# lxjeffffff/PagedAttention-Based-Transformer-Decoder-Inference-Framework

Measured on AMD Instinct MI355X. Metric: decode tokens/sec at batch=64 seq_len=8192; % HBM-roofline (1/2/4/8 GPU), higher is better.
Workload: dtype int8 GEMM (i32 acc) + fp16 KV attention (fp32 acc); 1 GPU; C3: INT8 decoder (MFMA i8 matmuls + fp16 paged attention), 24-layer/16-head/d=128, batch 64, KV context 8192, page 16; strong scaling: 64 rows over 1 GPU(s); global_batch=64, batch_per_gpu=64, seq_len=8192, page_size=16, parallelism=single GPU (no collective)

## Files before the change

pagedattention-based-transformer-decoder-inference-framework_amd/csrc/decoder.cpp:

```cpp
#include <algorithm>
#include <cmath>
#include <memory>
#include <mutex>
#include <random>
#include <string>
#include <vector>

#include "decoder_impl.hpp"

static int check_cfg(const llm_decoder_config& c) {
  LLM_REQUIRE(c.num_layers > 0 && c.num_heads > 0 && c.head_dim > 0 && c.vocab_size > 0 &&
                  c.max_seq_len > 0,
              "decoder: num_layers/num_heads/head_dim/vocab_size/max_seq_len must be positive");
  LLM_REQUIRE(c.hidden_dim == c.num_heads * c.head_dim,
              "decoder: hidden_dim must equal num_heads * head_dim");
  LLM_REQUIRE(c.weight_dtype == LLM_I8 || c.weight_dtype == LLM_F16, "decoder: weight_dtype");
  return LLM_OK;
}

static int create_decoder(const llm_decoder_config* cfg_in, int kv_dtype, llm_decoder** out) {
  LLM_REQUIRE(cfg_in && out, "llm_decoder_create: NULL");
  LLM_REQUIRE(kv_elem_size(kv_dtype) > 0, "llm_decoder_create_kv: unknown kv_dtype");
  if (kv_dtype != LLM_F16 && kv_dtype != LLM_FP8)
    return fail(LLM_ERR_UNSUPPORTED, "llm_decoder_create_kv: the decoder's KV pools are LLM_F16 "
// ... 33 lines not shown
  RET_IF(d->lm_pi.alloc((size_t)B * d->lm_nwg));
  RET_IF(d->sa.alloc((size_t)B));
  const size_t B16 = ((size_t)B + 15) / 16 * 16;
  RET_IF(d->qa.alloc(B16 * std::max(hid, inter)));
  if (d->wdtype == LLM_F16) {
    RET_IF(d->a16.alloc(2 * B16 * std::max(hid, inter)));
    RET_IF(d->oacc.alloc((size_t)B * hid));
    LLM_HIP_RET(hipMemset(d->oacc.p, 0, sizeof(long long) * B * hid));
    RET_IF(d->oflag.alloc(2));
    LLM_HIP_RET(hipMemset(d->oflag.p, 0, 2 * sizeof(int)));
    LLM_HIP_RET(hipHostMalloc(reinterpret_cast<void**>(&d->h_oflag), sizeof(int)));
    *d->h_oflag = 0;
  }
  RET_IF(d->beam_ctr.alloc(2 * (((size_t)B + 3) / 4) * d->H));
  LLM_HIP_RET(hipMemset(d->beam_ctr.p, 0, sizeof(unsigned) * d->beam_ctr.n));
  d->b16 = B16;
  RET_IF(d->tokens.alloc((size_t)B));
  RET_IF(d->beam_score.alloc((size_t)B));
  RET_IF(d->beam_ws.alloc(beam_select_ws_floats(B, 4)));
  RET_IF(d->cand_score.alloc((size_t)2 * B));
  RET_IF(d->cand_parent.alloc((size_t)2 * B));
  RET_IF(d->cand_token.alloc((size_t)2 * B));
  RET_IF(d->pos.alloc((size_t)B));
  RET_IF(d->ctx.alloc((size_t)B));
  d->pps = 0;
  d->attn_ws_bytes = 16;
  for (int b = 1; b <= B; ++b)
    d->attn_ws_bytes = std::max(d->attn_ws_bytes,
                                pa_decode_workspace_bytes(b, d->H, d->D, d->max_tiles, 0));
  RET_IF(d->attn_ws.alloc(std::max<size_t>(d->attn_ws_bytes, 16)));
// ... 84 lines not shown
  delete d;
}

extern "C" kv_cache* llm_decoder_kv(llm_decoder* d) { return d ? d->kv : nullptr; }

int llm::reset_rows(llm_decoder* d, int batch, int start_pos) {
  LLM_REQUIRE(batch > 0 && batch <= d->maxB, "decoder: batch must be in [1, max_batch]");
  RET_IF(kv_cache_clear(d->kv));
  d->batch = batch;
  if (d->row_group != 1) d->drop_step_graph();
  d->row_group = 1;
  d->h_pos.assign(d->maxB, 0);
  for (int b = 0; b < batch; ++b) d->h_pos[b] = start_pos;
  if (d->oacc.p) LLM_HIP_RET(hipMemset(d->oacc.p, 0, sizeof(long long) * d->oacc.n));
  if (d->oflag.p) LLM_HIP_RET(hipMemset(d->oflag.p, 0, sizeof(int)));
  d->range_clamped = 0;
  std::vector<int32_t> pos(batch, start_pos), ctx(batch, start_pos + 1), tok(batch, 0);
  LLM_HIP_RET(hipMemcpy(d->pos.p, pos.data(), sizeof(int32_t) * batch, hipMemcpyHostToDevice));
  LLM_HIP_RET(hipMemcpy(d->ctx.p, ctx.data(), sizeof(int32_t) * batch, hipMemcpyHostToDevice));
  LLM_HIP_RET(hipMemcpy(d->tokens.p, tok.data(), sizeof(int32_t) * batch, hipMemcpyHostToDevice));
  LLM_HIP_RET(hipDeviceSynchronize());
  return LLM_OK;
}

static void shuffle_free_pages(KvCache* k, uint64_t seed) {
  std::lock_guard<std::mutex> gk(k->mu);
  std::mt19937_64 rng(seed ^ 7);
  for (auto& f : k->free_lists) std::shuffle(f.begin(), f.end(), rng);
}

// ... 223 lines not shown
```

pagedattention-based-transformer-decoder-inference-framework_amd/csrc/decoder_impl.hpp:

```cpp
#pragma once

#include <mutex>
#include <string>
#include <unordered_map>
#include <vector>

#include "common.hpp"
#include "gemm.hpp"
#include "kv_cache_impl.hpp"
#include "pa_decode.hpp"
#include "row_ops.hpp"
#include "serve_plan.hpp"

using namespace llm;

namespace llm {

template <typename T>
struct __attribute__((visibility("hidden"))) DevBuf {
  T* p = nullptr;
  size_t n = 0;
  ~DevBuf() { if (p) (void)hipFree(p); }
  int alloc(size_t count) {
    if (p) { (void)hipFree(p); p = nullptr; }
// ... 14 lines not shown

struct Rows {
  int n = 0;
  float* x = nullptr;
  float* q = nullptr;
  float* o = nullptr;
  float* h1 = nullptr;
  void* act = nullptr;
  void* act2 = nullptr;
  float* sa = nullptr;
  const int32_t* pos = nullptr;
  const int32_t* ctx = nullptr;
  const int32_t* beam_rows = nullptr;
  int row_group = 1;
  bool wgm_quant = false;
  int prefill_row = -1;
  int prefill_p0 = 0;
  const int32_t* prefill_tiles = nullptr;
  int prefill_ntile = 0;
  int prefill_maxend = 0;
  bool is_prefill() const { return prefill_row >= 0 || prefill_ntile > 0; }
  uint8_t* attn_ws = nullptr;
  size_t attn_ws_bytes = 0;
  long long* oacc = nullptr;
  float* oproj_out = nullptr;
  int* oflag = nullptr;
};

struct llm_decoder {
  llm_decoder_config cfg{};
// ... 18 lines not shown
  DevBuf<float> rope;
  bool rope_on = false;
  int window = 0;

  DevBuf<float> x, qkv, o, h1, logits, sa;
  DevBuf<float> lm_pv;
  DevBuf<int32_t> lm_pi;
  int lm_nwg = 0;
  DevBuf<int8_t> qa;
  DevBuf<uint16_t> a16;
  DevBuf<long long> oacc, oacc_run;
  DevBuf<int> oflag, oflag_run;
  int* h_oflag = nullptr;
  int range_clamped = 0;
  DevBuf<unsigned> beam_ctr;
  int oproj_range_status();
  int report_range(int flag);
  DevBuf<int32_t> tokens, pos, ctx;
  DevBuf<uint8_t> attn_ws;
  size_t attn_ws_bytes = 0;

  int batch = 0;
  std::vector<int> h_pos;

  hipGraphExec_t graph = nullptr;
  int graph_batch{-1};
  void drop_step_graph() { graph_batch = -1; }

  int8_t* tap_q = nullptr;
  float* tap_s = nullptr;
// ... 15 lines not shown
  uint64_t sample_seed = 0;
  bool use_graph = true;
  bool beam_mode = false;
  DevBuf<float> beam_score, beam_ws, cand_score;
  DevBuf<int32_t> cand_parent, cand_token;
  std::vector<int32_t> h_cand;
  int qa_ld = 0;
  size_t b16 = 0;

  int layer_pre(int l, hipStream_t st, const Rows& R, const LnSource* emb = nullptr);
  int layer_attn(int l, hipStream_t st, const Rows& R);
  int attn_request(const Rows& R, pa_kv_view* view, PaRequest* rq, int l = 0);
  bool quant_prologue(const Rows& R) const;
  bool oproj_fusable(const Rows& R);
  bool wgm_quant_ok(const Rows& R);
  bool fc2_split(const Rows& R) const;
  int layer_post(int l, hipStream_t st, const Rows& R);
  int decode_rows(Rows* R, bool scratch_oproj = false);
  int next_tokens(const float* xr, int n, int r0, const int32_t* ctr, hipStream_t st,
                  int32_t* adv_pos = nullptr, int32_t* adv_ctx = nullptr);
  int enqueue_step(hipStream_t st);
  int run_step(const int32_t* tokens_host, float* logits_dev, int32_t* next_host, hipStream_t st);

  static constexpr int kPrefillChunk = 512;
  DevBuf<float> px, pq, po, ph1, psa;
  DevBuf<uint8_t> pact, pws;
  DevBuf<int32_t> pmeta;
  size_t pws_bytes = 0;
  int pf_cap = 0;
  int prefill_reserve(int C);
// ... 45 lines not shown
```

pagedattention-based-transformer-decoder-inference-framework_amd/csrc/decoder_serve.cpp:

```cpp
#include <cmath>
#include <mutex>
#include <string>
#include <vector>

#include "decoder_impl.hpp"

int llm_decoder::serve_upload() {
  const int n = plan.live();
  for (int r = 0; r < n; ++r) {
    const llm_request_options& o = requests.at(plan.row(r).id).opt;
    hs_temp[r] = o.temperature;
    hs_topk[r] = o.top_k;
    hs_topp[r] = o.top_p;
    hs_seed[r] = o.seed;
    hs_pos[r] = h_pos[r];
    hs_ctx[r] = h_pos[r] + 1;
  }
  auto up = [&](void* dst, const void* src, size_t bytes) {
    return hipMemcpyAsync(dst, src, bytes * n, hipMemcpyHostToDevice, stream);
  };
  LLM_HIP_RET(up(sv_temp.p, hs_temp.data(), sizeof(float)));
  LLM_HIP_RET(up(sv_topk.p, hs_topk.data(), sizeof(int32_t)));
  LLM_HIP_RET(up(sv_topp.p, hs_topp.data(), sizeof(float)));
  LLM_HIP_RET(up(sv_seed.p, hs_seed.data(), sizeof(uint64_t)));
// ... 70 lines not shown
  std::lock_guard<std::mutex> g(d->mu);
  LLM_REQUIRE(!d->serving, "llm_decoder_serve_begin: already serving");
  LLM_REQUIRE(d->weights_ready, "llm_decoder_serve_begin: weights not loaded");
  if (d->beam_mode)
    return fail(LLM_ERR_UNSUPPORTED, "llm_decoder_serve_begin: the decoder is in beam mode");
  if (d->V > 65536)
    return fail(LLM_ERR_UNSUPPORTED, "llm_decoder_serve_begin: vocab_size > 65536 (the rows' "
                                     "tokens are chosen by sample_rows_each)");
  LLM_HIP_RET(hipStreamSynchronize(d->stream));
  RET_IF(kv_cache_clear(d->kv));
  d->batch = 0;
  d->row_group = 1;
  d->h_pos.assign(d->maxB, 0);
  if (d->oacc.p) LLM_HIP_RET(hipMemset(d->oacc.p, 0, sizeof(long long) * d->oacc.n));
  if (d->oflag.p) LLM_HIP_RET(hipMemset(d->oflag.p, 0, sizeof(int)));
  LLM_HIP_RET(hipDeviceSynchronize());
  d->range_clamped = 0;
  const size_t B = (size_t)d->maxB;
  if (!d->sv_temp.p) {
    RET_IF(d->sv_temp.alloc(B));
    RET_IF(d->sv_topk.alloc(B));
    RET_IF(d->sv_topp.alloc(B));
    RET_IF(d->sv_seed.alloc(B));
  }
  d->hs_temp.assign(B, 0.f); d->hs_topp.assign(B, 1.f); d->hs_topk.assign(B, 0);
  d->hs_seed.assign(B, 0); d->hs_pos.assign(B, 0); d->hs_ctx.assign(B, 1);
  d->hs_tok.assign(B, 0); d->hs_next.assign(B, 0);
  ServeGeom geom;
  geom.max_rows = d->maxB;
  geom.num_pages = kv_cache_num_pages(d->kv);
// ... 92 lines not shown
```

pagedattention-based-transformer-decoder-inference-framework_amd/csrc/decoder_step.cpp:

```cpp
#include <mutex>
#include <string>

#include "decoder_impl.hpp"

__global__ void take_flag_kernel(int* f) { f[1] = atomicExch(f, 0); }

int llm_decoder::layer_pre(int l, hipStream_t st, const Rows& R, const LnSource* emb) {
  const size_t lh = (size_t)l * hid;
  pa_kv_view view;
  RET_IF(kv_cache_view(kv, l, &view));
  KvAppendView app;
  app.pos = R.pos;
  app.page_table = view.page_table;
  app.rows = R.beam_rows;
  app.k_pool = kv_cache_k_pool(kv);
  app.v_pool = kv_cache_v_pool(kv);
  app.num_beams = view.num_beams;
  app.max_tiles = view.max_tiles;
  app.page_size = TS;
  app.num_pages = view.num_pages;
  app.H = H;
  app.D = D;
  app.page_stride = (size_t)view.page_stride / kv_elem_size(kvt);
  app.kv_dtype = kvt;
// ... 56 lines not shown
  return attn_request(r, &view, &rq) == LLM_OK && pa_plan_device(rq, &p) == LLM_OK && p.oproj;
}

bool llm_decoder::wgm_quant_ok(const Rows& R) {
  if (wdtype != LLM_I8 || R.is_prefill() || R.row_group != 1 || R.beam_rows ||
      quant_prologue(R))
    return false;
  Rows r = R;
  r.wgm_quant = true;
  pa_kv_view view;
  PaRequest rq;
  PaLaunch p;
  return attn_request(r, &view, &rq) == LLM_OK && pa_plan_device(rq, &p) == LLM_OK && p.wgm;
}

bool llm_decoder::fc2_split(const Rows& R) const {
  return wdtype == LLM_I8 && !R.is_prefill() &&
         (R.n <= 16 || (R.n > 32 && R.n <= 64 && inter >= 16384)) &&
         !ln_fusable(wdtype, R.n, hid) && inter / 64 >= 16;
}

int llm_decoder::attn_request(const Rows& R, pa_kv_view* view, PaRequest* rq, int l) {
  RET_IF(kv_cache_view(kv, l, view));
  const PaOut out = quant_prologue(R) || R.wgm_quant ? PaOut::F32_ROWS
                    : wdtype == LLM_I8               ? PaOut::ROW_Q
                    : R.oacc                         ? PaOut::OPROJ
                                                     : PaOut::ROW_F16;
  *rq = pa_request(view, R.n, H, D, cfg.max_seq_len, pps, R.row_group, out);
  rq->rows16 = out == PaOut::OPROJ && tap_q;
  rq->steal_ctr = R.row_group >= 4 && beam_steal_on();
  rq->window = window;
  return LLM_OK;
}

int llm_decoder::layer_attn(int l, hipStream_t st, const Rows& R) {
  pa_kv_view view;
  PaRequest rq;
  RET_IF(attn_request(R, &view, &rq, l));
  PaRowOutputs ro;
  ro.pack = 1;
  ro.keep_out = 0;
  if (rq.out == PaOut::ROW_Q) {
    ro.q = static_cast<int8_t*>(R.act);
    ro.inv_scale = R.sa;
  } else if (rq.out == PaOut::OPROJ) {
    ro.o_acc = R.oacc;
    ro.o_x = R.oproj_out;
    ro.wo_heads = wo_heads.p + (size_t)l * hid * hid;
    ro.o_n = hid;
    ro.o_flag = R.oflag;
    ro.out16 = rq.rows16 ? R.act : nullptr;
  } else if (rq.out == PaOut::ROW_F16) {
    ro.out16 = R.act;
  }
  if (rq.steal_ctr) ro.beam_ctr = beam_ctr.p;
  ro.out_scale = v_scale[l];
  const float sm = kvt == LLM_FP8 ? cfg.attn_scale * k_scale[l] : cfg.attn_scale;
  if (R.is_prefill() && pa_prefill_supported(&view)) {
    if (R.prefill_ntile > 0)
// ... 9 lines not shown
    LLM_HIP_RET(launch_quantize_rows(R.o, R.n, hid, static_cast<int8_t*>(R.act), R.sa, st, 1));
  return LLM_OK;
}

int llm_decoder::layer_post(int l, hipStream_t st, const Rows& R) {
  const size_t lh = (size_t)l * hid;
  const bool i8 = wdtype == LLM_I8;
  WeightGemm g;
  g.dtype = wdtype;
  g.a_packed = 1;
  g.w_keep = w_keep;
  g.A = R.act;
  g.M = R.n;
  g.W_packed = wo.p + sz_o * l; g.N = hid; g.K = hid; g.C = R.x;
  if (i8) { g.sa = R.sa; g.sw = sw_o.p + lh; }
  const bool qpro = quant_prologue(R);
  if (qpro) {
    g.ln_x = R.o;
    g.ln_quant_only = 1;
    if (tap_q) { g.act_out = R.act; g.sa_out = R.sa; }
  }
  if (!R.oacc) RET_IF(weight_gemm(g, st));
  g.ln_x = nullptr; g.ln_quant_only = 0; g.act_out = nullptr; g.sa_out = nullptr;
  RET_IF(tap(l, 1, R, hid, st));
  const bool split_fc2 = fc2_split(R);
  RET_IF(layer_norm_into(g, R, ln2_g.p + lh, ln2_b.p + lh, st, split_fc2 ? R.x : nullptr));
  g.W_packed = w1.p + sz_1 * l; g.N = inter; g.K = hid;
  g.bias = b1.p + (size_t)l * inter; g.act = LLM_ACT_RELU;
  if (i8) {
    g.C = R.h1;
    g.sw = sw1.p + (size_t)l * inter;
// ... 27 lines not shown
  R.ctx = ctx.p;
  R.row_group = row_group;
  R.attn_ws = attn_ws.p;
  R.attn_ws_bytes = attn_ws_bytes;
  if (oproj_fusable(R)) {
    if (scratch_oproj && !oacc_run.p) {
      RET_IF(oacc_run.alloc(oacc.n));
      LLM_HIP_RET(hipMemset(oacc_run.p, 0, sizeof(long long) * oacc_run.n));
      RET_IF(oflag_run.alloc(1));
      LLM_HIP_RET(hipMemset(oflag_run.p, 0, sizeof(int)));
    }
    R.oacc = scratch_oproj ? oacc_run.p : oacc.p;
    R.oproj_out = scratch_oproj ? R.o : R.x;
    R.oflag = scratch_oproj ? oflag_run.p : oflag.p;
  }
  R.wgm_quant = wgm_quant_ok(R);
  return LLM_OK;
}

int llm_decoder::tap(int l, int stage, const Rows& R, int K, hipStream_t st) {
  if (!tap_q || R.is_prefill() || R.beam_rows) return LLM_OK;
  const bool f16 = wdtype == LLM_F16;
  const size_t es = f16 ? 2 : 1;
  const size_t slot = (size_t)l * 4 + stage;
  const size_t n16 = ((size_t)R.n + 15) / 16 * 16;
  const void* src = f16 && stage == 3 ? R.act2 : R.act;
  LLM_HIP_RET(hipMemcpyAsync(tap_q + slot * b16 * qa_ld * es, src, n16 * K * es,
                             hipMemcpyDeviceToDevice, st));
  if (!f16)
    LLM_HIP_RET(hipMemcpyAsync(tap_s + slot * maxB, R.sa, sizeof(float) * R.n,
                               hipMemcpyDeviceToDevice, st));
// ... 139 lines not shown
```

pagedattention-based-transformer-decoder-inference-framework_amd/csrc/pa_decode.hip:

```cpp
#include "pa_split.hpp"

namespace llm {

struct PaMergeRowArgs {
  const float* part_acc;
  const float* part_ml;
  float* out;
  int8_t* q;
  float* inv_scale;
  _Float16* out16;
  const int32_t* context_lens;
  int B, H, D, T, TS, pps, nsplit, max_tiles;
  int pack;
  int ctx_p0;
  float out_scale;
  int window;
};

template <int DPL, int BATCH>
__device__ __forceinline__ float merge_head(const float* ml, const float* pa, int nsplit, int ns,
                                            int D, float (&acc)[DPL]) {
  const int lane = lane_id();
  const int nsl = max(nsplit - 1, 0);
  const float m0r = ml[2 * min(lane, nsl)], l0r = ml[2 * min(lane, nsl) + 1];
// ... 207 lines not shown
namespace {


template <int D, int TS, PaSplitCfg C>
hipError_t launch_form(const PaSplitArgs& a, dim3 grid, dim3 block, hipStream_t st) {
  hipLaunchKernelGGL((pa_split_kernel<D, TS, C>), grid, block, 0, st, a);
  return hipGetLastError();
}

template <int D, int TS, int KVT>
hipError_t launch_split(const PaSplitArgs& a, const PaLaunch& p, hipStream_t st) {
  const int waves = ((a.B + a.group - 1) / a.group) * a.group * a.H * a.nsplit;
  const dim3 grid((waves + 3) / 4), block(256);
  if (p.wgm) {
    const dim3 wgrid(a.B * a.H), wblock(64 * a.nsplit);
    if constexpr (KVT == LLM_F16) {
      if constexpr (D <= kOprojMaxD) {
        if (p.oproj) return launch_form<D, TS, pa_cfg_wgm_oproj(D, TS)>(a, wgrid, wblock, st);
      }
      return launch_form<D, TS, pa_cfg_wgm(D, TS)>(a, wgrid, wblock, st);
    } else if constexpr (KVT == LLM_FP8 && fp8_wgm_shape_ok(D, TS)) {
      return launch_form<D, TS, pa_cfg_wgm_fp8(D, TS)>(a, wgrid, wblock, st);
    } else {
      return hipErrorInvalidValue;
    }
  }
  if constexpr (KVT == LLM_F16) {
    if (p.beam) {
      hipError_t te;
      if (tune_launch_form(a, D, TS, grid, st, &te)) return te;
// ... 5 lines not shown
}

bool supported(int D, int TS, int kvt) {
  return pa_for_shape(D, TS, kvt, false, [](auto, auto, auto) { return true; });
}

}

int pa_plan_device(const PaRequest& rq, PaLaunch* launch, long long resident,
                   long long beam_resident, long long beam4_resident) {
  *launch = PaLaunch{};
  const int D = rq.D, TS = rq.TS;
  if (!supported(D, TS, rq.kv_dtype)) return LLM_ERR_UNSUPPORTED;
  const PaTuning tn = pa_tuning();
  const bool beam_group = rq.row_group == 4 && rq.kv_dtype == LLM_F16;
  if (rq.pps_fixed > 0) {
    resident = beam_resident = beam4_resident = 0;
  } else {
    if (resident < 0)
      resident = pa_for_shape(D, TS, rq.kv_dtype, kFallbackResident, [](auto d, auto ts, auto k) {
        return resident_waves<decltype(d)::value, decltype(ts)::value, decltype(k)::value>();
      });
    if (beam_resident < 0)
      beam_resident = !beam_group ? 0 : pa_for_shape(D, TS, LLM_F16, 0LL, [](auto d, auto ts, auto) {
        return beam_resident_waves<decltype(d)::value, decltype(ts)::value>();
      });
    if (beam4_resident < 0)
      beam4_resident = beam_group && tn.beam4 && !tn.beam_mfma && split_stages(D, TS, 2) == 2
                           ? tune_beam4_resident_for(D, TS) : 0;
  }
  return pa_plan(rq, tn, resident, beam_resident, beam4_resident, launch);
}

int pa_pages_per_split(int B, int H, int T, int TS, int max_tiles) {
  const int ntiles = std::max(1, std::min((T + TS - 1) / TS, max_tiles));
  const int ns = choose_nsplit(B, H, ntiles, 0, kFallbackResident);
  return (ntiles + ns - 1) / ns;
}


}

using namespace llm;

extern "C" int pa_decode_pages_per_split(int B, int H, int T, int page_size, int max_tiles) {
  if (B < 0 || H <= 0 || T < 0 || page_size <= 0 || max_tiles <= 0) return -1;
// ... 129 lines not shown
  a.balance16 = tn.beam_balance16;
  a.smaj = a.group == 4 && tn.beam_smaj ? 1 : 0;
  a.beam4 = p.beam4 ? 1 : 0;
  if (p.steal && a.group == 4)
    a.steal = rows && rows->beam_ctr ? rows->beam_ctr
                                     : tune_steal_counters(2 * (size_t)((B + 3) / 4) * H);
  if (p.wgm) {
    a.wgm = 1;
    a.out16 = rows ? static_cast<_Float16*>(rows->out16) : nullptr;
    a.pack = rows ? rows->pack : 0;
    a.out = f32_rows || (rows && rows->keep_out) ? out : nullptr;
    if (oproj) {
      a.o_acc = rows->o_acc, a.o_x = rows->o_x, a.o_n = rows->o_n, a.o_flag = rows->o_flag;
      a.wo_heads = static_cast<const _Float16*>(rows->wo_heads);
    }
  }
  const hipError_t e =
      pa_for_shape(D, TS, kv->kv_dtype, hipErrorInvalidValue, [&](auto d, auto ts, auto k) {
        return launch_split<decltype(d)::value, decltype(ts)::value, decltype(k)::value>(a, p, st);
      });
  if (e != hipSuccess) return fail(LLM_ERR_HIP, std::string("pa_split launch: ") + hipGetErrorString(e));
  if (p.wgm) return LLM_OK;
  if (row_out && !p.direct)
    return pa_merge_rows_internal(a.part_acc, a.part_ml, rows->keep_out ? out : nullptr, rows,
                                  context_lens, -1, B, H, D, T, TS, p.beam ? -1 : p.pps, p.nsplit,
                                  kv->max_tiles, st, out_scale, rq.window);
  if (!p.direct) {
    const int r = pa_merge_splits_internal(a.part_acc, a.part_ml, out, context_lens, B, H, D, T,
                                           TS, p.beam ? -1 : p.pps, p.nsplit, kv->max_tiles, st,
                                           out_scale, rq.window);
// ... 67 lines not shown
```

pagedattention-based-transformer-decoder-inference-framework_amd/csrc/pa_decode.hpp:

```cpp
#pragma once

#include <hip/hip_runtime.h>

#include "llm_decoder.h"
#include "pa_plan.hpp"

namespace llm {

struct PaRowOutputs {
  int8_t* q = nullptr;
  float* inv_scale = nullptr;
  void* out16 = nullptr;
  int pack = 0;
  int keep_out = 1;
  long long* o_acc = nullptr;
  float* o_x = nullptr;
  const void* wo_heads = nullptr;
  int o_n = 0;
  int* o_flag = nullptr;
  unsigned* beam_ctr = nullptr;
  float out_scale = 1.f;
};

constexpr int kv_elem_size(int kvt) {
  return kvt == LLM_F16 || kvt == LLM_BF16 ? 2
         : kvt == LLM_F32                  ? 4
         : kvt == LLM_I8 || kvt == LLM_FP8 ? 1
                                           : 0;
}

inline PaRequest pa_request(const pa_kv_view* kv, int B, int H, int D, int T, int pages_per_split,
                            int row_group = 1, PaOut out = PaOut::F32, int window = 0) {
  PaRequest rq;
  rq.B = B, rq.H = H, rq.D = D, rq.T = T;
  if (kv) rq.TS = kv->page_size, rq.max_tiles = kv->max_tiles, rq.kv_dtype = kv->kv_dtype;
// ... 52 lines not shown
```

pagedattention-based-transformer-decoder-inference-framework_amd/csrc/pa_plan.hpp:

```cpp
#pragma once

#include <algorithm>

#include "llm_decoder.h"
#include "pa_tuning.hpp"

namespace llm {

constexpr int kWgmMaxSplits = 8;
constexpr int kOprojMaxD = 128;

constexpr int kMaxPps = 128;
constexpr int kMaxSplits = 128;
constexpr int kMinPps = 8;
constexpr int kMaxWavesPerCu = 32;
constexpr long long kFallbackResident = 256LL * 4 * 3;

constexpr int split_stages(int D, int TS, int es) { return TS * D * es > 8192 ? 1 : 2; }

constexpr bool fp8_wgm_shape_ok(int D, int TS) { return D * TS <= 2048; }

enum class PaOut {
  F32,
  ROW_Q,
  ROW_F16,
  F32_ROWS,
  OPROJ,
};

struct PaRequest {
  int B = 0, H = 0, D = 0, T = 0, TS = 0, max_tiles = 0;
  int kv_dtype = LLM_F16;
  int pps_fixed = 0;
  int row_group = 1;
  PaOut out = PaOut::F32;
  bool rows16 = false;
  bool steal_ctr = false;
  bool keep_out = true;
  int window = 0;
};

struct PaLaunch {
  int nsplit = 0;
  int pps = 0;
  bool direct = false, wgm = false, beam = false, beam4 = false, steal = false, oproj = false;
  bool steal_ctr = false;
  bool merge_row = false;
  size_t workspace_bytes = 0;
  int form() const {
    if (nsplit <= 0) return 0;
    return (direct ? LLM_PA_FORM_DIRECT : wgm ? LLM_PA_FORM_WG_MERGE
            : merge_row ? LLM_PA_FORM_SPLIT_MERGE_ROW : LLM_PA_FORM_SPLIT_MERGE) |
           (beam ? LLM_PA_FORM_BEAM : 0) | (oproj ? LLM_PA_FORM_OPROJ : 0) |
           (steal && steal_ctr ? LLM_PA_FORM_STEAL : 0);
  }
};

inline long long max_nsplit(int B, int H, int ntiles) {
  ntiles = std::max(ntiles, 1);
  const long long bh = std::max(1LL, (long long)B * H);
  const long long cap = 256LL * kMaxWavesPerCu;
  const long long lo = (ntiles + kMaxPps - 1) / kMaxPps;
// ... 15 lines not shown
  const long long bh = std::max(1LL, (long long)B * H);
  const long long lo = (ntiles + kMaxPps - 1) / kMaxPps;
  long long ns = lo;
  for (long long k = 1; k <= 64; ++k) {
    const long long cand = (k * resident + bh - 1) / bh;
    if (cand >= lo) { ns = cand; break; }
  }
  ns = std::min<long long>(ns, std::max(1, (ntiles + kMinPps - 1) / kMinPps));
  if ((ntiles + ns - 1) / ns < short_pps)
    ns = std::min(ns, std::max<long long>((ntiles + short_pps - 1) / short_pps,
                                          (kMinLaunchWaves + bh - 1) / bh));
  ns = std::max(ns, lo);
  return (int)std::min(ns, max_nsplit(B, H, ntiles));
}

inline int pa_plan(const PaRequest& rq, const PaTuning& tn, long long resident,
                   long long beam_resident, long long beam4_resident, PaLaunch* out) {
  const int B = rq.B, H = rq.H, D = rq.D, TS = rq.TS, row_group = rq.row_group, kvt = rq.kv_dtype;
  const bool oproj = rq.out == PaOut::OPROJ, f32_rows = rq.out == PaOut::F32_ROWS;
  const bool out16 = rq.out == PaOut::ROW_F16 || (oproj && rq.rows16);
  int ntiles_max = std::max(1, std::min((rq.T + TS - 1) / TS, rq.max_tiles));
  if (rq.window > 0) ntiles_max = std::min(ntiles_max, (rq.window - 1) / TS + 2);
  *out = PaLaunch{};
  if (rq.window > 0 && row_group > 1) return LLM_ERR_UNSUPPORTED;
  const int pps_fixed = rq.pps_fixed > 0 ? std::min(rq.pps_fixed, kMaxPps) : 0;
  const bool beam_shape = kvt == LLM_F16 && split_stages(D, TS, 2) == 2;
  const long long resident_launch =
      pps_fixed <= 0 && row_group == 4 && kvt == LLM_F16 ? std::max(resident, beam_resident)
                                                         : resident;
  int nsplit = choose_nsplit(B, H, ntiles_max, pps_fixed, resident_launch);
  const bool half_round = f32_rows && row_group == 1 && pps_fixed <= 0 &&
                          (kvt == LLM_F16 || kvt == LLM_FP8) &&
                          nsplit > kWgmMaxSplits &&
                          (long long)B * H * nsplit == resident_launch &&
// ... 36 lines not shown
  if (nsplit > kMaxSplits || (long long)nsplit * (pps_fixed > 0 ? pps_fixed : kMaxPps) < ntiles_max)
    return LLM_ERR_UNSUPPORTED;
  const int group = std::max(1, std::min(row_group, 4));
  PaLaunch p;
  p.nsplit = nsplit;
  p.pps = pps_fixed;
  p.direct = nsplit <= 1;
  p.wgm = wgm_ok && !p.direct && group == 1 && nsplit <= kWgmMaxSplits;
  p.oproj = oproj && p.wgm;
  p.beam = group == 4 && !p.direct && beam_shape;
  p.beam4 = use_beam4;
  p.steal = tn.beam_steal && row_group >= 4 && !p.direct && kvt == LLM_F16 && pps_fixed <= 0 &&
            !use_beam4 && !tn.beam_mfma && steal_shape_ok(D, TS);
  p.steal_ctr = rq.steal_ctr;
  p.merge_row = rq.out == PaOut::ROW_Q || out16;
  p.workspace_bytes =
      p.direct || p.wgm ? 0 : (size_t)B * H * nsplit * (size_t)(D + 2) * sizeof(float);
  *out = p;
  return LLM_OK;
}

}
```

pagedattention-based-transformer-decoder-inference-framework_amd/csrc/pa_split.hpp:

```cpp
#pragma once

#include "common.hpp"
#include "ln_wave.hpp"
#include "pa_decode.hpp"
#include "row_ops.hpp"

#include <algorithm>
#include <type_traits>
#include <cstdlib>

namespace llm {

struct PaSplitArgs {
  const uint8_t* k_pool;
  const uint8_t* v_pool;
  const int32_t* page_table;
  const float* q;
  int q_stride;
  float* out;
  float* part_acc;
  float* part_ml;
  const int32_t* beam_ids;
  const int32_t* context_lens;
  int B, H, T;
// ... 6 lines not shown
  int balance16;
  _Float16* out16;
  int pack;
  int wgm;
  int beam4;
  long long* o_acc;
  float* o_x;
  const _Float16* wo_heads;
  int o_n;
  int* o_flag;
  unsigned* steal;
  unsigned long long* stamps;
  int smaj;
  float out_scale;
  int window;
};

__device__ __forceinline__ int row_pps(int pps_fixed, int nsplit, int ntiles) {
  if (pps_fixed > 0) return pps_fixed;
  return min(max((ntiles + nsplit - 1) / nsplit, 1), kMaxPps);
}

struct PaSpan {
  int t_lo, lo_tile, n_live;
};
__device__ __forceinline__ PaSpan row_span(int Tb, int ntiles, int window, int TS) {
  const int t_lo = window > 0 ? max(0, Tb - window) : 0;
  const int lo_tile = t_lo / TS;
  return {t_lo, lo_tile, max(ntiles - lo_tile, 0)};
}
__device__ __forceinline__ int row_nsplits(int pps_fixed, int nsplit, int n_live) {
// ... 39 lines not shown
  bool direct = false;
  int chunk_bytes = 16384;
  int aux = kKvLoadAux;
  int stages = 2;
  int min_waves = 0;
  bool load_only = false;
  bool beam = false;
  int kvt = LLM_F16;
  bool fullpath = true;
  bool wgm = false;
  bool oproj = false;
  int ring = 0;
  bool stamps = false;
  bool interleave = false;
  bool prio = false;
};

template <int D, int TS, PaSplitCfg C>
__global__ __launch_bounds__(C.wgm ? 64 * kWgmMaxSplits : 256)
__attribute__((amdgpu_waves_per_eu(C.min_waves > 0 ? C.min_waves : 1)))
void pa_split_kernel(PaSplitArgs a) {
  constexpr int ES = kv_elem_bytes<C.kvt>();
  constexpr int EPL = 16 / ES;
  constexpr int LPT = D / EPL;
  constexpr int TPI = 64 / LPT;
  constexpr int NI = TS / TPI;
  constexpr int PAGE_BYTES = TS * D * ES;
  constexpr int U = pages_per_stage<PAGE_BYTES, C.chunk_bytes>();
  constexpr int NR = U * NI;
  static_assert(LPT >= 1 && LPT <= 64 && TS % TPI == 0 && NI >= 1, "bad D/TS");

  static_assert(!(C.wgm && (C.direct || C.beam)), "the workgroup merge is a split form");
  static_assert(!C.interleave || C.beam, "interleaved splits are a beam-group form");
  constexpr bool IL = C.beam && C.interleave;
  static_assert(!C.oproj || (C.wgm && C.kvt == LLM_F16), "the fused o_proj is a workgroup-merge form");
  const unsigned long long t_entry = C.stamps ? __builtin_amdgcn_s_memrealtime() : 0ull;
  if constexpr (C.beam && C.prio) __builtin_amdgcn_s_setprio(3);
  const int lane = lane_id();
  const int wid = blockIdx.x * (C.wgm ? a.nsplit : 4) + wave_id_uniform();
  const int G = C.beam ? 4 : C.wgm ? 1 : a.group;
  const int gi = wid % G;
  const int rest = wid / G;
  const int GH = C.beam && a.smaj ? ((a.B + 3) / 4) * a.H : 1;
  const int s = C.beam && a.smaj ? rest / GH : rest % a.nsplit;
  const int gh = C.beam && a.smaj ? rest % GH : rest / a.nsplit;
  const int h = gh % a.H;
  const int b = (gh / a.H) * G + gi;
  constexpr int kPfx = 512;
  bool share = false;
  int grow[4] = {0, 0, 0, 0};
// ... 463 lines not shown
        float inv = 1.0f / (L + 1e-6f);
        if constexpr (C.kvt == LLM_FP8) inv *= a.out_scale;
        float am[EPL];
#pragma unroll
        for (int e = 0; e < EPL; ++e) am[e] = 0.f;
#pragma unroll
        for (int s2 = 0; s2 < kWgmMaxSplits; ++s2) {
          const float ws = __int_as_float(__builtin_amdgcn_readlane(__float_as_int(w0), s2));
          const float* src = &wg_acc[min(s2, max(ns - 1, 0))][c * EPL];
#pragma unroll
          for (int e = 0; e < EPL; ++e) am[e] += src[e] * ws;
        }
#pragma unroll
        for (int e = 0; e < EPL; ++e) o[e] = am[e] * inv;
      }
      if (lane < LPT) {
        const int hid = a.H * D;
        const int k0 = h * D + c * EPL;
        if (a.out) {
          float* op = a.out + (size_t)b * hid + k0;
#pragma unroll
          for (int e = 0; e < EPL; e += 4) *reinterpret_cast<f32x4*>(op + e) = f32x4{o[e], o[e + 1], o[e + 2], o[e + 3]};
        }
        if (a.out16) {
          static_assert(C.kvt != LLM_F16 || EPL == 8, "fp16 lanes hold 8 dims: one 16-byte store");
          if constexpr (EPL == 8) {
            f16x8 pk;
#pragma unroll
            for (int e = 0; e < 8; ++e) pk[e] = (_Float16)o[e];
            *reinterpret_cast<f16x8*>(a.out16 + (a.pack ? a_frag_off_f16(b, k0, hid >> 5)
// ... 81 lines not shown
      unsigned hw = 0, xcc = 0;
      asm volatile("s_getreg_b32 %0, hwreg(HW_REG_HW_ID)" : "=s"(hw));
      asm volatile("s_getreg_b32 %0, hwreg(HW_REG_XCC_ID)" : "=s"(xcc));
      st[4] = ((unsigned long long)xcc << 32) | hw;
    }
  }
}

constexpr PaSplitCfg pa_cfg_split(int D, int TS, int kvt, bool direct = false) {
  return {.direct = direct, .stages = split_stages(D, TS, kv_elem_size(kvt)), .kvt = kvt};
}
constexpr PaSplitCfg pa_cfg_wgm(int D, int TS, int kvt = LLM_F16) {
  return {.stages = split_stages(D, TS, kv_elem_size(kvt)), .kvt = kvt, .wgm = true};
}
constexpr PaSplitCfg pa_cfg_wgm_fp8(int D, int TS) { return pa_cfg_wgm(D, TS, LLM_FP8); }
constexpr PaSplitCfg pa_cfg_wgm_oproj(int D, int TS) {
  return {.stages = split_stages(D, TS, 2), .wgm = true, .oproj = true};
}
#ifndef LLM_BEAM_CHUNK
#define LLM_BEAM_CHUNK 8192
#define LLM_BEAM_WAVES 0
#endif
constexpr PaSplitCfg pa_cfg_beam() {
  return {.chunk_bytes = LLM_BEAM_CHUNK, .min_waves = LLM_BEAM_WAVES, .beam = true,
          .interleave = true, .prio = true};
}

template <class R, class F>
R pa_for_shape(int D, int TS, int kvt, R unsupported, F&& f) {
  auto by_ts = [&](auto d, auto k) -> R {
// ... 44 lines not shown
```

pagedattention-based-transformer-decoder-inference-framework_amd/csrc/pa_tuning.hpp:

```cpp
#pragma once

namespace llm {

struct PaTuning {
  bool wg_merge = true;
  bool oproj_fuse = true;
  bool beam4 = false;
  bool beam_mfma = false;
  bool beam_steal = false;
  int beam_balance16 = 44;
  int beam_mfma_balance16 = 64;
  int beam_nsplit = 0;
  int wgm_splits = 0;
  int beam4_splits = 0;
  bool beam_smaj = true;
};

constexpr bool steal_shape_ok(int D, int TS) {
  return D >= 8 && D <= 512 && (TS * D) % 1024 == 0 && TS * D * 2 <= 8192;
}

#if LLM_TUNING
PaTuning pa_tuning();
#else
constexpr PaTuning pa_tuning() { return PaTuning{}; }
#endif

}
```

pagedattention-based-transformer-decoder-inference-framework_amd/csrc/tune/pa_decode_tune.hip:

```cpp
#include <cmath>

#include "tune/pa_decode_tune.hpp"
#include "tune/pa_beam_steal.hpp"
#include "beam_plan.hpp"
#include "pa_tuning.hpp"
#include "prefill_pack.hpp"
#include "serve_plan.hpp"

namespace llm {

template <int D, int TS, int MINW = 2, int U = 1>
__global__ __launch_bounds__(256) __attribute__((amdgpu_waves_per_eu(MINW))) void pa_beam4_kernel(PaSplitArgs a) {
  constexpr int G = 4;
  constexpr int EPL = 8;
  constexpr int LPT = D / EPL;
  constexpr int TPI = 64 / LPT;
  constexpr int NI = TS / TPI;
  constexpr int PAGE_BYTES = TS * D * 2;
  static_assert(LPT >= 1 && LPT <= 64 && TS % TPI == 0 && NI >= 1 && PAGE_BYTES <= 8192,
                "pa_beam4_kernel: fp16 pages of 1..8 KiB");
  const int lane = lane_id();
  const int wid = blockIdx.x * 4 + wave_id_uniform();
  const int s = wid % a.nsplit;
  const int gh = wid / a.nsplit;
// ... 716 lines not shown
    const int x = env_int("LLM_BEAM_MFMA_BALANCE16", 64);
    return x >= 16 ? x : 0;
  }();
  PaTuning t;
  t.wg_merge = env_int("LLM_WG_MERGE", 1) != 0;
  t.oproj_fuse = env_int("LLM_OPROJ_FUSE", 1) != 0;
  t.beam4 = env_int("LLM_BEAM4", 0) != 0;
  t.beam_mfma = env_int("LLM_BEAM_MFMA", 0) != 0;
  t.beam_steal = env_int("LLM_BEAM_STEAL", 0) == 1;
  t.beam_balance16 = balance;
  t.beam_mfma_balance16 = mfma_balance;
  t.beam_nsplit = env_int("LLM_BEAM_NSPLIT", 0);
  t.wgm_splits = env_int("LLM_WGM_SPLITS", 0);
  t.beam4_splits = env_int("LLM_BEAM4_SPLITS", 0);
  t.beam_smaj = env_int("LLM_BEAM_SMAJ", 1) != 0;
  return t;
}

bool tune_beam_occupancy(int D, int TS, int* blocks, hipError_t* e) {
  if (D != 128 || TS != 16 || !pa_tuning().beam_mfma) return false;
  *e = tune_beam_mfma_occupancy(blocks);
  return true;
}

unsigned* tune_steal_counters(size_t n) {
  static unsigned* buf = nullptr;
  static size_t cap = 0;
  if (!pa_tuning().beam_steal) return nullptr;
  if (n > cap) {
    if (buf) (void)hipFree(buf);
// ... 123 lines not shown
  if (rc != LLM_OK) return rc;
  if (pa_plan_device(rq, &p, resident, beam_resident, beam4_resident) != LLM_OK)
    return fail(LLM_ERR_UNSUPPORTED, "pa_plan_window_tune: more splits than a row may have");
  *nsplit = p.nsplit;
  *form = p.form();
  return LLM_OK;
}

extern "C" int pa_plan_tune(int B, int H, int D, int T, int page_size, int max_tiles, int kv_dtype,
                            int pages_per_split, int row_group, int out_kind, int rows16,
                            long long resident, long long beam_resident, long long beam4_resident,
                            int* nsplit, int* form) {
  return pa_plan_window_tune(B, H, D, T, page_size, max_tiles, kv_dtype, pages_per_split, row_group,
                             0, out_kind, rows16, resident, beam_resident, beam4_resident, nsplit,
                             form);
}

extern "C" int prefill_passes_tune(const int32_t* start, const int32_t* len, int nrows, int cap,
                                   int32_t* out, int capacity) {
  if (nrows < 0 || cap < 1 || capacity < 0 || (nrows && (!start || !len)) || (capacity && !out))
    return -1;
  for (int i = 0; i < nrows; ++i)
    if (start[i] < 0 || len[i] < 0) return -1;
  int n = 0, pi = 0;
  for (const PrefillPass& pass : prefill_passes(start, len, nrows, cap)) {
    for (const PrefillSeg& s : pass) {
      if (n < capacity) {
        int32_t* q = out + 4 * (size_t)n;
        q[0] = pi, q[1] = s.src, q[2] = s.p0, q[3] = s.len;
      }
// ... 152 lines not shown
```

Baseline: 3789 tokens/s.

## Fuse per-row int8 quantisation into workgroup-merge attention via last-head counter

Adds a workgroup-merge attention variant that writes fp32 head outputs and then atomically counts finished heads per row. The last workgroup for a row quantises the whole row to int8 with its scale, directly in the packed layout the o_proj GEMM expects. This removes the separate quantisation prologue in the o_proj GEMM, along with the extra pass over the attention output. In exchange it adds per-row atomics, a memory fence, and a serial tail in which one wave quantises each row. It applies only when the hidden size is at most 4096 and the resulting grid fits within the resident-wave budget.

```diff
diff --git a/pagedattention-based-transformer-decoder-inference-framework_amd/csrc/decoder.cpp b/pagedattention-based-transformer-decoder-inference-framework_amd/csrc/decoder.cpp
--- a/pagedattention-based-transformer-decoder-inference-framework_amd/csrc/decoder.cpp
+++ b/pagedattention-based-transformer-decoder-inference-framework_amd/csrc/decoder.cpp
@@ -71,6 +71,10 @@
   }
   RET_IF(d->beam_ctr.alloc(2 * (((size_t)B + 3) / 4) * d->H));
   LLM_HIP_RET(hipMemset(d->beam_ctr.p, 0, sizeof(unsigned) * d->beam_ctr.n));
+  if (d->wdtype == LLM_I8) {
+    RET_IF(d->row_ctr.alloc(2 * (size_t)B));
+    LLM_HIP_RET(hipMemset(d->row_ctr.p, 0, sizeof(int) * d->row_ctr.n));
+  }
   d->b16 = B16;
   RET_IF(d->tokens.alloc((size_t)B));
   RET_IF(d->beam_score.alloc((size_t)B));
@@ -185,6 +189,7 @@
   for (int b = 0; b < batch; ++b) d->h_pos[b] = start_pos;
   if (d->oacc.p) LLM_HIP_RET(hipMemset(d->oacc.p, 0, sizeof(long long) * d->oacc.n));
   if (d->oflag.p) LLM_HIP_RET(hipMemset(d->oflag.p, 0, sizeof(int)));
+  if (d->row_ctr.p) LLM_HIP_RET(hipMemset(d->row_ctr.p, 0, sizeof(int) * d->row_ctr.n));
   d->range_clamped = 0;
   std::vector<int32_t> pos(batch, start_pos), ctx(batch, start_pos + 1), tok(batch, 0);
   LLM_HIP_RET(hipMemcpy(d->pos.p, pos.data(), sizeof(int32_t) * batch, hipMemcpyHostToDevice));
diff --git a/pagedattention-based-transformer-decoder-inference-framework_amd/csrc/decoder_impl.hpp b/pagedattention-based-transformer-decoder-inference-framework_amd/csrc/decoder_impl.hpp
--- a/pagedattention-based-transformer-decoder-inference-framework_amd/csrc/decoder_impl.hpp
+++ b/pagedattention-based-transformer-decoder-inference-framework_amd/csrc/decoder_impl.hpp
@@ -52,6 +52,7 @@
   const int32_t* beam_rows = nullptr;
   int row_group = 1;
   bool wgm_quant = false;
+  int* row_ctr = nullptr;
   int prefill_row = -1;
   int prefill_p0 = 0;
   const int32_t* prefill_tiles = nullptr;
@@ -100,6 +101,7 @@
   int* h_oflag = nullptr;
   int range_clamped = 0;
   DevBuf<unsigned> beam_ctr;
+  DevBuf<int> row_ctr;
   int oproj_range_status();
   int report_range(int flag);
   DevBuf<int32_t> tokens, pos, ctx;
@@ -145,6 +147,7 @@
   bool quant_prologue(const Rows& R) const;
   bool oproj_fusable(const Rows& R);
   bool wgm_quant_ok(const Rows& R);
+  bool rowq_ok(const Rows& R);
   bool fc2_split(const Rows& R) const;
   int layer_post(int l, hipStream_t st, const Rows& R);
   int decode_rows(Rows* R, bool scratch_oproj = false);
diff --git a/pagedattention-based-transformer-decoder-inference-framework_amd/csrc/decoder_serve.cpp b/pagedattention-based-transformer-decoder-inference-framework_amd/csrc/decoder_serve.cpp
--- a/pagedattention-based-transformer-decoder-inference-framework_amd/csrc/decoder_serve.cpp
+++ b/pagedattention-based-transformer-decoder-inference-framework_amd/csrc/decoder_serve.cpp
@@ -108,6 +108,7 @@
   d->h_pos.assign(d->maxB, 0);
   if (d->oacc.p) LLM_HIP_RET(hipMemset(d->oacc.p, 0, sizeof(long long) * d->oacc.n));
   if (d->oflag.p) LLM_HIP_RET(hipMemset(d->oflag.p, 0, sizeof(int)));
+  if (d->row_ctr.p) LLM_HIP_RET(hipMemset(d->row_ctr.p, 0, sizeof(int) * d->row_ctr.n));
   LLM_HIP_RET(hipDeviceSynchronize());
   d->range_clamped = 0;
   const size_t B = (size_t)d->maxB;
diff --git a/pagedattention-based-transformer-decoder-inference-framework_amd/csrc/decoder_step.cpp b/pagedattention-based-transformer-decoder-inference-framework_amd/csrc/decoder_step.cpp
--- a/pagedattention-based-transformer-decoder-inference-framework_amd/csrc/decoder_step.cpp
+++ b/pagedattention-based-transformer-decoder-inference-framework_amd/csrc/decoder_step.cpp
@@ -94,6 +94,16 @@
   return attn_request(r, &view, &rq) == LLM_OK && pa_plan_device(rq, &p) == LLM_OK && p.wgm;
 }
 
+bool llm_decoder::rowq_ok(const Rows& R) {
+  if (!row_ctr.p || R.beam_rows || !(quant_prologue(R) || wgm_quant_ok(R))) return false;
+  Rows r = R;
+  r.row_ctr = row_ctr.p;
+  pa_kv_view view;
+  PaRequest rq;
+  PaLaunch p;
+  return attn_request(r, &view, &rq) == LLM_OK && pa_plan_device(rq, &p) == LLM_OK && p.rowq;
+}
+
 bool llm_decoder::fc2_split(const Rows& R) const {
   return wdtype == LLM_I8 && !R.is_prefill() &&
          (R.n <= 16 || (R.n > 32 && R.n <= 64 && inter >= 16384)) &&
@@ -102,13 +112,15 @@
 
 int llm_decoder::attn_request(const Rows& R, pa_kv_view* view, PaRequest* rq, int l) {
   RET_IF(kv_cache_view(kv, l, view));
-  const PaOut out = quant_prologue(R) || R.wgm_quant ? PaOut::F32_ROWS
+  const PaOut out = R.row_ctr                        ? PaOut::ROW_Q
+                    : quant_prologue(R) || R.wgm_quant ? PaOut::F32_ROWS
                     : wdtype == LLM_I8               ? PaOut::ROW_Q
                     : R.oacc                         ? PaOut::OPROJ
                                                      : PaOut::ROW_F16;
   *rq = pa_request(view, R.n, H, D, cfg.max_seq_len, pps, R.row_group, out);
   rq->rows16 = out == PaOut::OPROJ && tap_q;
   rq->steal_ctr = R.row_group >= 4 && beam_steal_on();
+  rq->row_ctr = R.row_ctr != nullptr;
   rq->window = window;
   return LLM_OK;
 }
@@ -123,6 +135,7 @@
   if (rq.out == PaOut::ROW_Q) {
     ro.q = static_cast<int8_t*>(R.act);
     ro.inv_scale = R.sa;
+    ro.row_ctr = R.row_ctr;
   } else if (rq.out == PaOut::OPROJ) {
     ro.o_acc = R.oacc;
     ro.o_x = R.oproj_out;
@@ -162,7 +175,7 @@
   g.M = R.n;
   g.W_packed = wo.p + sz_o * l; g.N = hid; g.K = hid; g.C = R.x;
   if (i8) { g.sa = R.sa; g.sw = sw_o.p + lh; }
-  const bool qpro = quant_prologue(R);
+  const bool qpro = quant_prologue(R) && !R.row_ctr;
   if (qpro) {
     g.ln_x = R.o;
     g.ln_quant_only = 1;
@@ -220,7 +233,10 @@
     R.oproj_out = scratch_oproj ? R.o : R.x;
     R.oflag = scratch_oproj ? oflag_run.p : oflag.p;
   }
-  R.wgm_quant = wgm_quant_ok(R);
+  if (rowq_ok(R))
+    R.row_ctr = row_ctr.p + (scratch_oproj ? maxB : 0);
+  else
+    R.wgm_quant = wgm_quant_ok(R);
   return LLM_OK;
 }
 
diff --git a/pagedattention-based-transformer-decoder-inference-framework_amd/csrc/pa_decode.hip b/pagedattention-based-transformer-decoder-inference-framework_amd/csrc/pa_decode.hip
--- a/pagedattention-based-transformer-decoder-inference-framework_amd/csrc/pa_decode.hip
+++ b/pagedattention-based-transformer-decoder-inference-framework_amd/csrc/pa_decode.hip
@@ -245,6 +245,9 @@
   const dim3 grid((waves + 3) / 4), block(256);
   if (p.wgm) {
     const dim3 wgrid(a.B * a.H), wblock(64 * a.nsplit);
+    if constexpr (KVT == LLM_F16 || (KVT == LLM_FP8 && fp8_wgm_shape_ok(D, TS))) {
+      if (p.rowq) return launch_form<D, TS, pa_cfg_wgm_rowq(D, TS, KVT)>(a, wgrid, wblock, st);
+    }
     if constexpr (KVT == LLM_F16) {
       if constexpr (D <= kOprojMaxD) {
         if (p.oproj) return launch_form<D, TS, pa_cfg_wgm_oproj(D, TS)>(a, wgrid, wblock, st);
@@ -280,6 +283,12 @@
   if (!supported(D, TS, rq.kv_dtype)) return LLM_ERR_UNSUPPORTED;
   const PaTuning tn = pa_tuning();
   const bool beam_group = rq.row_group == 4 && rq.kv_dtype == LLM_F16;
+  long long rowq_round = 0;
+  if (rq.out == PaOut::ROW_Q && rq.row_ctr)
+    rowq_round = resident >= 0 ? resident
+                               : pa_for_shape(D, TS, rq.kv_dtype, kFallbackResident, [](auto d, auto ts, auto k) {
+                                   return resident_waves<decltype(d)::value, decltype(ts)::value, decltype(k)::value>();
+                                 });
   if (rq.pps_fixed > 0) {
     resident = beam_resident = beam4_resident = 0;
   } else {
@@ -295,7 +304,7 @@
       beam4_resident = beam_group && tn.beam4 && !tn.beam_mfma && split_stages(D, TS, 2) == 2
                            ? tune_beam4_resident_for(D, TS) : 0;
   }
-  return pa_plan(rq, tn, resident, beam_resident, beam4_resident, launch);
+  return pa_plan(rq, tn, resident, beam_resident, beam4_resident, launch, rowq_round);
 }
 
 int pa_pages_per_split(int B, int H, int T, int TS, int max_tiles) {
@@ -455,6 +464,13 @@
       a.o_acc = rows->o_acc, a.o_x = rows->o_x, a.o_n = rows->o_n, a.o_flag = rows->o_flag;
       a.wo_heads = static_cast<const _Float16*>(rows->wo_heads);
     }
+    if (p.rowq) {
+      LLM_REQUIRE(out && rows->row_ctr && rows->pack && !rows->out16,
+                  "pa_decode: in-launch row quantisation needs the fp32 rows, row counters and "
+                  "packed q");
+      a.out = out;
+      a.row_q = rows->q, a.row_inv = rows->inv_scale, a.row_ctr = rows->row_ctr;
+    }
   }
   const hipError_t e =
       pa_for_shape(D, TS, kv->kv_dtype, hipErrorInvalidValue, [&](auto d, auto ts, auto k) {
diff --git a/pagedattention-based-transformer-decoder-inference-framework_amd/csrc/pa_decode.hpp b/pagedattention-based-transformer-decoder-inference-framework_amd/csrc/pa_decode.hpp
--- a/pagedattention-based-transformer-decoder-inference-framework_amd/csrc/pa_decode.hpp
+++ b/pagedattention-based-transformer-decoder-inference-framework_amd/csrc/pa_decode.hpp
@@ -19,6 +19,7 @@
   int o_n = 0;
   int* o_flag = nullptr;
   unsigned* beam_ctr = nullptr;
+  int* row_ctr = nullptr;
   float out_scale = 1.f;
 };
 
diff --git a/pagedattention-based-transformer-decoder-inference-framework_amd/csrc/pa_plan.hpp b/pagedattention-based-transformer-decoder-inference-framework_amd/csrc/pa_plan.hpp
--- a/pagedattention-based-transformer-decoder-inference-framework_amd/csrc/pa_plan.hpp
+++ b/pagedattention-based-transformer-decoder-inference-framework_amd/csrc/pa_plan.hpp
@@ -9,6 +9,7 @@
 
 constexpr int kWgmMaxSplits = 8;
 constexpr int kOprojMaxD = 128;
+constexpr int kRowqMaxHid = 4096;
 
 constexpr int kMaxPps = 128;
 constexpr int kMaxSplits = 128;
@@ -37,6 +38,7 @@
   bool rows16 = false;
   bool steal_ctr = false;
   bool keep_out = true;
+  bool row_ctr = false;
   int window = 0;
 };
 
@@ -46,6 +48,7 @@
   bool direct = false, wgm = false, beam = false, beam4 = false, steal = false, oproj = false;
   bool steal_ctr = false;
   bool merge_row = false;
+  bool rowq = false;
   size_t workspace_bytes = 0;
   int form() const {
     if (nsplit <= 0) return 0;
@@ -91,10 +94,10 @@
   return (int)std::min(ns, max_nsplit(B, H, ntiles));
 }
 
-inline int pa_plan(const PaRequest& rq, const PaTuning& tn, long long resident,
-                   long long beam_resident, long long beam4_resident, PaLaunch* out) {
+inline int pa_plan_as(const PaRequest& rq, const PaTuning& tn, long long resident,
+                      long long beam_resident, long long beam4_resident, bool rowq, PaLaunch* out) {
   const int B = rq.B, H = rq.H, D = rq.D, TS = rq.TS, row_group = rq.row_group, kvt = rq.kv_dtype;
-  const bool oproj = rq.out == PaOut::OPROJ, f32_rows = rq.out == PaOut::F32_ROWS;
+  const bool oproj = rq.out == PaOut::OPROJ, f32_rows = rq.out == PaOut::F32_ROWS || rowq;
   const bool out16 = rq.out == PaOut::ROW_F16 || (oproj && rq.rows16);
   int ntiles_max = std::max(1, std::min((rq.T + TS - 1) / TS, rq.max_tiles));
   if (rq.window > 0) ntiles_max = std::min(ntiles_max, (rq.window - 1) / TS + 2);
@@ -161,10 +164,24 @@
             !use_beam4 && !tn.beam_mfma && steal_shape_ok(D, TS);
   p.steal_ctr = rq.steal_ctr;
   p.merge_row = rq.out == PaOut::ROW_Q || out16;
+  p.rowq = rowq && p.wgm;
   p.workspace_bytes =
       p.direct || p.wgm ? 0 : (size_t)B * H * nsplit * (size_t)(D + 2) * sizeof(float);
   *out = p;
   return LLM_OK;
 }
 
+inline int pa_plan(const PaRequest& rq, const PaTuning& tn, long long resident,
+                   long long beam_resident, long long beam4_resident, PaLaunch* out,
+                   long long rowq_round = 0) {
+  if (rq.out == PaOut::ROW_Q && rq.row_ctr && tn.rowq && rq.row_group == 1 &&
+      (long long)rq.H * rq.D <= kRowqMaxHid && (rq.H * rq.D) % 64 == 0) {
+    const int rc = pa_plan_as(rq, tn, resident, beam_resident, beam4_resident, true, out);
+    if (rc == LLM_OK && out->rowq &&
+        (rowq_round <= 0 || (long long)rq.B * rq.H * out->nsplit <= rowq_round))
+      return rc;
+  }
+  return pa_plan_as(rq, tn, resident, beam_resident, beam4_resident, false, out);
 }
+
+}
diff --git a/pagedattention-based-transformer-decoder-inference-framework_amd/csrc/pa_split.hpp b/pagedattention-based-transformer-decoder-inference-framework_amd/csrc/pa_split.hpp
--- a/pagedattention-based-transformer-decoder-inference-framework_amd/csrc/pa_split.hpp
+++ b/pagedattention-based-transformer-decoder-inference-framework_amd/csrc/pa_split.hpp
@@ -44,7 +44,37 @@
   int smaj;
   float out_scale;
   int window;
+  int8_t* row_q;
+  float* row_inv;
+  int* row_ctr;
 };
+
+template <int CPL>
+__device__ __forceinline__ void rowq_finish(const float* row, int hid, int b, int8_t* q,
+                                            float* inv_scale) {
+  const int lane = lane_id();
+  const int K4 = hid >> 2;
+  const auto rs = __builtin_amdgcn_make_buffer_rsrc((void*)row, (short)0, hid * 4, 0x00020000);
+  LnRow<CPL> x;
+#pragma unroll
+  for (int j = 0; j < CPL; ++j)
+    x.v[j] = __builtin_bit_cast(
+        f32x4, __builtin_amdgcn_raw_buffer_load_b128(rs, (uint32_t)(64 * j + lane) * 16u, 0, 16));
+  float am = 0.f;
+#pragma unroll
+  for (int j = 0; j < CPL; ++j)
+#pragma unroll
+    for (int e = 0; e < 4; ++e) am = fmaxf(am, fabsf(x.v[j][e]));
+  am = ln_wave_max(am);
+  const float scale = 127.f / (am + 1e-6f);
+#pragma unroll
+  for (int j = 0; j < CPL; ++j) {
+    const int c = 64 * j + lane;
+    if (c < K4)
+      *reinterpret_cast<uint32_t*>(q + a_frag_off_i8(b, 4 * c, hid >> 6)) = ln_quant4(x.v[j], scale);
+  }
+  if (lane == 0) inv_scale[b] = 1.0f / scale;
+}
 
 __device__ __forceinline__ int row_pps(int pps_fixed, int nsplit, int ntiles) {
   if (pps_fixed > 0) return pps_fixed;
@@ -114,6 +144,7 @@
   bool stamps = false;
   bool interleave = false;
   bool prio = false;
+  bool rowq = false;
 };
 
 template <int D, int TS, PaSplitCfg C>
@@ -134,6 +165,7 @@
   static_assert(!C.interleave || C.beam, "interleaved splits are a beam-group form");
   constexpr bool IL = C.beam && C.interleave;
   static_assert(!C.oproj || (C.wgm && C.kvt == LLM_F16), "the fused o_proj is a workgroup-merge form");
+  static_assert(!C.rowq || (C.wgm && !C.oproj), "the in-launch row quantisation is a workgroup-merge form");
   const unsigned long long t_entry = C.stamps ? __builtin_amdgcn_s_memrealtime() : 0ull;
   if constexpr (C.beam && C.prio) __builtin_amdgcn_s_setprio(3);
   const int lane = lane_id();
@@ -627,6 +659,32 @@
 #pragma unroll
         for (int e = 0; e < EPL; ++e) o[e] = am[e] * inv;
       }
+      if constexpr (C.rowq) {
+        const int hid = a.H * D;
+        float* orow = a.out + (size_t)b * hid;
+        if (lane < LPT) {
+          const auto ors = __builtin_amdgcn_make_buffer_rsrc((void*)orow, (short)0, hid * 4, 0x00020000);
+#pragma unroll
+          for (int e = 0; e < EPL; e += 4)
+            __builtin_amdgcn_raw_buffer_store_b128(
+                __builtin_bit_cast(u32x4, f32x4{o[e], o[e + 1], o[e + 2], o[e + 3]}), ors,
+                (uint32_t)(h * D + c * EPL + e) * 4u, 0, 16);
+        }
+        asm volatile("s_waitcnt vmcnt(0)" ::: "memory");
+        int t = 0;
+        if (lane == 0)
+          t = __hip_atomic_fetch_add(a.row_ctr + b, 1, __ATOMIC_RELAXED, __HIP_MEMORY_SCOPE_AGENT);
+        t = __builtin_amdgcn_readfirstlane(t);
+        if (t != a.H - 1) return;
+        if (lane == 0)
+          __hip_atomic_store(a.row_ctr + b, 0, __ATOMIC_RELAXED, __HIP_MEMORY_SCOPE_AGENT);
+        __builtin_amdgcn_fence(__ATOMIC_ACQUIRE, "agent");
+        if (hid <= 2048)
+          rowq_finish<8>(orow, hid, b, a.row_q, a.row_inv);
+        else
+          rowq_finish<16>(orow, hid, b, a.row_q, a.row_inv);
+        return;
+      }
       if (lane < LPT) {
         const int hid = a.H * D;
         const int k0 = h * D + c * EPL;
@@ -738,6 +796,11 @@
   return {.stages = split_stages(D, TS, kv_elem_size(kvt)), .kvt = kvt, .wgm = true};
 }
 constexpr PaSplitCfg pa_cfg_wgm_fp8(int D, int TS) { return pa_cfg_wgm(D, TS, LLM_FP8); }
+constexpr PaSplitCfg pa_cfg_wgm_rowq(int D, int TS, int kvt) {
+  PaSplitCfg c = pa_cfg_wgm(D, TS, kvt);
+  c.rowq = true;
+  return c;
+}
 constexpr PaSplitCfg pa_cfg_wgm_oproj(int D, int TS) {
   return {.stages = split_stages(D, TS, 2), .wgm = true, .oproj = true};
 }
diff --git a/pagedattention-based-transformer-decoder-inference-framework_amd/csrc/pa_tuning.hpp b/pagedattention-based-transformer-decoder-inference-framework_amd/csrc/pa_tuning.hpp
--- a/pagedattention-based-transformer-decoder-inference-framework_amd/csrc/pa_tuning.hpp
+++ b/pagedattention-based-transformer-decoder-inference-framework_amd/csrc/pa_tuning.hpp
@@ -14,6 +14,7 @@
   int wgm_splits = 0;
   int beam4_splits = 0;
   bool beam_smaj = true;
+  bool rowq = true;
 };
 
 constexpr bool steal_shape_ok(int D, int TS) {
diff --git a/pagedattention-based-transformer-decoder-inference-framework_amd/csrc/tune/pa_decode_tune.hip b/pagedattention-based-transformer-decoder-inference-framework_amd/csrc/tune/pa_decode_tune.hip
--- a/pagedattention-based-transformer-decoder-inference-framework_amd/csrc/tune/pa_decode_tune.hip
+++ b/pagedattention-based-transformer-decoder-inference-framework_amd/csrc/tune/pa_decode_tune.hip
@@ -754,6 +754,7 @@
   t.wgm_splits = env_int("LLM_WGM_SPLITS", 0);
   t.beam4_splits = env_int("LLM_BEAM4_SPLITS", 0);
   t.beam_smaj = env_int("LLM_BEAM_SMAJ", 1) != 0;
+  t.rowq = env_int("LLM_PA_ROWQ", 1) != 0;
   return t;
 }
 
@@ -907,6 +908,45 @@
   return pa_plan_window_tune(B, H, D, T, page_size, max_tiles, kv_dtype, pages_per_split, row_group,
                              0, out_kind, rows16, resident, beam_resident, beam4_resident, nsplit,
                              form);
+}
+
+extern "C" int pa_plan_rowq_tune(int B, int H, int D, int T, int page_size, int max_tiles,
+                                 int kv_dtype, int pages_per_split, int window, long long resident,
+                                 int* nsplit, int* form, int* rowq) {
+  LLM_REQUIRE(nsplit && form && rowq, "pa_plan_rowq_tune: NULL output");
+  *nsplit = *form = *rowq = 0;
+  pa_kv_view kv{};
+  kv.num_heads = H, kv.head_dim = D, kv.page_size = page_size, kv.max_tiles = max_tiles;
+  kv.kv_dtype = kv_dtype;
+  PaRequest rq = pa_request(&kv, B, H, D, T, pages_per_split, 1, PaOut::ROW_Q, window);
+  rq.row_ctr = true;
+  PaLaunch p;
+  if (pa_plan_device(rq, &p, resident, 0, 0) != LLM_OK)
+    return fail(LLM_ERR_UNSUPPORTED, "pa_plan_rowq_tune: no plan");
+  *nsplit = p.nsplit;
+  *form = p.form();
+  *rowq = p.rowq ? 1 : 0;
+  return LLM_OK;
+}
+
+extern "C" int pa_decode_rowq_tune(const pa_kv_view* kv, const float* q, float* out,
+                                   const int32_t* context_lens, int B, int H, int T,
+                                   float sm_scale, int pages_per_split, int window,
+                                   float out_scale, int8_t* q8, float* inv_scale, int* row_ctr,
+                                   void* workspace, size_t workspace_bytes, int* rowq,
+                                   void* stream) {
+  LLM_REQUIRE(kv && q8 && inv_scale && row_ctr && rowq, "pa_decode_rowq_tune: NULL");
+  PaRequest rq = pa_request(kv, B, H, kv->head_dim, T, pages_per_split, 1, PaOut::ROW_Q, window);
+  rq.row_ctr = true;
+  PaLaunch p;
+  if (pa_plan_device(rq, &p) != LLM_OK) return fail(LLM_ERR_UNSUPPORTED, "pa_decode_rowq_tune: no plan");
+  *rowq = p.rowq ? 1 : 0;
+  PaRowOutputs ro;
+  ro.q = q8, ro.inv_scale = inv_scale, ro.pack = 1, ro.keep_out = 1;
+  ro.row_ctr = row_ctr;
+  ro.out_scale = out_scale;
+  return pa_decode_internal(kv, rq, q, H * kv->head_dim, out, nullptr, context_lens, sm_scale,
+                            workspace, workspace_bytes, as_stream(stream), &ro);
 }
 
 extern "C" int prefill_passes_tune(const int32_t* start, const int32_t* len, int nrows, int cap,
```

Result: no change. 3789 tokens/s (median of 6 runs) (+0.0%).
